# Pasqui1010/DART-Planner

Hardware: AMD Instinct MI355X
Metric: SE(3) rollouts/sec (N=30, batch=8192) + p95 solve ms, at 1/2/4/8 MI355X (higher is better)
Workload: dtype f32

## Files before the change

### dart_planner_amd/capi.py

```python
from __future__ import annotations

import ctypes as C
import math
import os
from typing import Optional

_HERE = os.path.dirname(os.path.abspath(__file__))
DEFAULT_LIBRARY = os.path.join(_HERE, "libse3mpc.so")

SE3MPC_MAX_HORIZON = 64
SE3MPC_MAX_CORRECTIONS = 10
SE3MPC_MAX_SPHERES = 256

STATUS_NAMES = {0: "SE3MPC_OK", -1: "SE3MPC_ERR_NULL", -2: "SE3MPC_ERR_HORIZON", -3: "SE3MPC_ERR_SHAPE",
                -4: "SE3MPC_ERR_PARAM", -5: "SE3MPC_ERR_WORKSPACE", -6: "SE3MPC_ERR_LAUNCH",
                -7: "SE3MPC_ERR_NO_DEVICE"}
TASK_MESSAGES = {1: "CONVERGENCE: NORM OF PROJECTED GRADIENT <= PGTOL",
                 2: "CONVERGENCE: RELATIVE REDUCTION OF F <= FACTR*EPSMCH",
                 3: "STOP: TOTAL NO. OF ITERATIONS REACHED LIMIT",
                 4: "STOP: TOTAL NO. OF F,G EVALUATIONS EXCEEDS LIMIT",
                 5: "ABNORMAL: "}


class Se3mpcLibraryError(RuntimeError):
# ... 285 lines not shown
    "mixer_readback": [_XP, _I, _P, _P, _LL, _P, _P, _P, _P, _P, _P],
    "closed_loop_actuated": [_MP, _CP, _SP, _XP, _I, _I, _D] + _PLAN + [_P, _P, _P, _P, _P, _P, _P, _P, _P, _LL, _P, _LL, _I,
                             C.POINTER(C.c_double * 3), _P, _P, _P, _P, _P, _P, _P],
    "latency_push": [_I, _I, _P, _P, _P, _P, _P, _P, _P, _P, _P, _P, _P, _P, _P, _P],
    "onboard_control": [_OP, _I, _P, _P, _P, _P] + _PLAN + [_P, _P, _P, _P, _P],
    "edge_loop": [_OP, _SP, _I, _I, _D] + _PLAN + [_P, _P, _P, _P, _P, _P, _I, _P, _P, _P, _P, _LL, _I, C.POINTER(C.c_double * 3),
                  _P, _P, _P, _P, _P, _P, _P],
    "monte_carlo": [_PP, _CP, _SP, _I, _I, _I, _D, _P, _P, _LL, _P, _P, _P, _P, _P, _P, _P, _P, _P, _P, _P],
    "monte_carlo_staged": [_PP, _CP, _SP, _MP, _XP, _I, _I, _I, _D, _P, _P, _LL, _P, _P, _P, _P, _P, _P, _P, _P, _P, _LL, _P, _P, _P, _P, _P],
    "mppi_closed_loop": [_PP, _CP, _SP, _I, _I, _I, _D, C.c_uint32, _I, _I, _I, _D, _D, C.c_uint64, C.c_uint32, C.c_uint32, _P, _P, _I, _D, _P, _LL,
                         _P, _P, _P, _P, _P, _P, _P, _P, _P, _P, _P, _P],
    "mppi_closed_loop_staged": [_PP, _CP, _SP, _MP, _XP, _I, _I, _I, _D, C.c_uint32, _I, _I, _I, _D, _D, C.c_uint64, C.c_uint32, C.c_uint32, _P, _P, _I,
                                _D, _P, _LL, _P, _P, _P, _P, _P, _P, _P, _P, _P, _LL, _P, _P, _P, _P, _P, _P, _P],
}
_PLAIN_API = {
    "se3mpc_controller_default_params": (C.c_int, [_CP]),
    "se3mpc_simulator_default_params": (C.c_int, [_SP]),
    "se3mpc_controller_reset": (C.c_int, [_CP, _I, _P, _P]),
    "se3mpc_smoother_default_params": (C.c_int, [_MP]),
    "se3mpc_smoother_reset": (C.c_int, [_I, _P, _P]),
    "se3mpc_mixer_default_params": (C.c_int, [_XP]),
    "se3mpc_mixer_reset": (C.c_int, [_I, _P, _P]),
    "se3mpc_onboard_default_params": (C.c_int, [_OP]),
    "se3mpc_onboard_reset": (C.c_int, [_I, _P, _P]),
    "se3mpc_latency_reset": (C.c_int, [_I, _I, _P, _P]),
    "se3mpc_abi_version": (C.c_int, []),
    "se3mpc_last_error": (C.c_char_p, []),
    "se3mpc_device_count": (C.c_int, []),
    "se3mpc_default_params": (C.c_int, [_PP]),
    "se3mpc_check_params": (C.c_int, [_PP]),
    "se3mpc_set_rollout_variant": (C.c_int, [_I]),
    "se3mpc_set_solver_variant": (C.c_int, [_I]),
    "se3mpc_set_edge_loop_variant": (C.c_int, [_I]),
    "se3mpc_reduce_keys": (C.c_int, [_P, _I, _I, _P, _P]),
    "se3mpc_key_index": (C.c_uint32, [C.c_uint64]),
    "se3mpc_key_cost": (C.c_float, [C.c_uint64]),
    "se3mpc_population_workspace": (C.c_int, [_I, _I]),
    "se3mpc_mppi_split_workspace_bytes": (C.c_size_t, [_I, _I, _I]),
}


def exported_symbols() -> list:
    names = list(_PLAIN_API)
    for base in _TYPED_API:
        names += [f"se3mpc_{base}_f32", f"se3mpc_{base}_f64"]
    for base in _LOOP_TYPED_API:
        names += [f"se3mpc_{base}_f32", f"se3mpc_{base}_f64"]
    names += list(_VOXEL_PLAIN_API)
    for base in _VOXEL_TYPED_API:
        names += [f"se3mpc_voxel_{base}_f32", f"se3mpc_voxel_{base}_f64"]
    return names


class Library:

    def __init__(self, path: Optional[str] = None):
        self.path = path or os.environ.get("SE3MPC_LIBRARY", DEFAULT_LIBRARY)
        if not os.path.exists(self.path):
            raise Se3mpcLibraryError(
                f"{self.path} not found: the HIP extension has not been built.  Run "
                "`python -c 'import __graft_entry__ as g; g.build()'` (or `make -C dart_planner_amd/csrc`). "
                "There is no CPU fallback.")
        try:
            self._dll = C.CDLL(self.path)
        except OSError as e:
            raise Se3mpcLibraryError(f"cannot load {self.path}: {e}") from e
# ... 19 lines not shown
            for suf in ("f32", "f64"):
                fn = getattr(self._dll, f"se3mpc_voxel_{base}_{suf}")
                fn.restype = C.c_int
                fn.argtypes = [_VP] + args
        if self._dll.se3mpc_abi_version() != 1:
            raise Se3mpcLibraryError(f"{self.path}: ABI version {self._dll.se3mpc_abi_version()} != 1")

    def abi_version(self) -> int:
        return self._dll.se3mpc_abi_version()

    def last_error(self) -> str:
        return (self._dll.se3mpc_last_error() or b"").decode()

    def device_count(self) -> int:
        return self._dll.se3mpc_device_count()

    def default_params(self) -> Params:
        p = Params()
        self._check("se3mpc_default_params", self._dll.se3mpc_default_params(C.byref(p)))
        return p

    def check_params(self, p: Params) -> int:
        return self._dll.se3mpc_check_params(C.byref(p))

    def set_rollout_variant(self, variant: int) -> None:
        self._check("se3mpc_set_rollout_variant", self._dll.se3mpc_set_rollout_variant(variant))

    def set_solver_variant(self, variant: int) -> None:
        self._check("se3mpc_set_solver_variant", self._dll.se3mpc_set_solver_variant(variant))

    def set_edge_loop_variant(self, variant: int) -> None:
        self._check("se3mpc_set_edge_loop_variant", self._dll.se3mpc_set_edge_loop_variant(variant))

    def reduce_keys(self, wave_keys: int, per_batch: int, nbatch: int, keys_out: int, stream: int) -> None:
        self._check("se3mpc_reduce_keys", self._dll.se3mpc_reduce_keys(wave_keys, per_batch, nbatch, keys_out, stream))

    def population_workspace(self, rows: int, B: int) -> int:
        return self._dll.se3mpc_population_workspace(rows, B)

    def mppi_split_workspace_bytes(self, horizon: int, nprob: int, splits: int) -> int:
        return self._dll.se3mpc_mppi_split_workspace_bytes(horizon, nprob, splits)

    def key_index(self, key: int) -> int:
        return self._dll.se3mpc_key_index(C.c_uint64(key))

    def key_cost(self, key: int) -> float:
        return self._dll.se3mpc_key_cost(C.c_uint64(key))

    def call(self, base: str, suffix: str, *args, params: Optional[Params] = None) -> None:
        fn = getattr(self._dll, f"se3mpc_{base}_{suffix}")
        has_params = _TYPED_API[base][0]
        if has_params:
            if params is None:
                raise TypeError(f"se3mpc_{base} needs params")
            rc = fn(C.byref(params), *args)
        else:
            rc = fn(*args)
        self._check(f"se3mpc_{base}_{suffix}", rc)

    def call_status(self, base: str, suffix: str, *args, params: Optional[Params] = None) -> int:
        fn = getattr(self._dll, f"se3mpc_{base}_{suffix}")
        if _TYPED_API[base][0]:
            return fn(C.byref(params) if params is not None else None, *args)
        return fn(*args)

    def controller_default_params(self) -> ControllerParams:
# ... 74 lines not shown
```

### dart_planner_amd/csrc/closed_loop.hip

```cpp
#pragma clang fp contract(off)
#include "closed_loop_device.hpp"

namespace se3mpc {

template <typename R>
__global__ void __launch_bounds__(64)
control_kernel(CtrlDev<R> c, int B, const double* __restrict__ time, const R* __restrict__ pos, const R* __restrict__ vel,
               const R* __restrict__ att, const R* __restrict__ omega, const R* __restrict__ dpos, const R* __restrict__ dvel,
               const R* __restrict__ dacc, const R* __restrict__ yaw, const R* __restrict__ yaw_rate, double* __restrict__ state,
               R* __restrict__ thrust, R* __restrict__ torque, R* __restrict__ body_thrust, R* __restrict__ body_rates,
               int32_t* __restrict__ flags, const double* __restrict__ sample_time, PlanView<R> plan, R* __restrict__ target) {
  const int b = blockIdx.x * blockDim.x + threadIdx.x;
  if (b >= B) return;
  CtrlRegs<R> s = load_ctrl<R>(state + (size_t)b * SE3MPC_CONTROLLER_STATE_WORDS);
  DroneRegs<R> d;
  d.load_state(b, pos, vel, att, omega);
  R dp[3], dv[3], da[3];
  if (sample_time != nullptr) {
    const PlanView<R> rows = plan.of(b);
    PlanCursor<R> cur;
    cursor_reset(cur);
    sample_plan<R>(sample_time[b], plan.N, rows.ts, rows.P, rows.V, rows.A, dp, dv, da, cur);
    if (target != nullptr) for (int i = 0; i < 3; ++i) { target[9 * b + i] = dp[i]; target[9 * b + 3 + i] = dv[i]; target[9 * b + 6 + i] = da[i]; }
  } else {
// ... 88 lines not shown
  if (cos_angle != nullptr) cos_angle[b] = ca;
  if (singular != nullptr) singular[b] = sing ? 1 : 0;
}

template <typename R>
__global__ void __launch_bounds__(64)
closed_loop_kernel(CtrlDev<R> c, SimDev<R> m, int B, int nsteps, double sim_dt, PlanView<R> plan, double* __restrict__ time,
                   R* __restrict__ pos, R* __restrict__ vel, R* __restrict__ att, R* __restrict__ omega, double* __restrict__ state,
                   const R* __restrict__ wind, long long wind_stride, int gust_step, R gx, R gy, R gz, int stop_at_plan_end,
                   R* __restrict__ log_state, R* __restrict__ log_cmd, double* __restrict__ log_time, int32_t* __restrict__ steps_taken) {
  const int b = blockIdx.x * blockDim.x + threadIdx.x;
  if (b >= B) return;
  CtrlRegs<R> s = load_ctrl<R>(state + (size_t)b * SE3MPC_CONTROLLER_STATE_WORDS);
  DroneRegs<R> d;
  d.load(b, pos, vel, att, omega, wind, wind_stride, time);
  const int N = plan.N;
  const PlanView<R> rows = plan.of(b);
  const double* __restrict__ ts = rows.ts;
  const R* __restrict__ Pb = rows.P;
  const R* __restrict__ Vb = rows.V;
  const R* __restrict__ Ab = rows.A;
  const R dt = (R)sim_dt;
  PlanCursor<R> cur;
  cursor_reset(cur);
  const int taken = lane_loop<R>(d, b, B, nsteps, gust_step, gx, gy, gz, stop_at_plan_end != 0, ts[N - 1], log_state, log_cmd, log_time,
                                 [&](int, R& th, R* tq) { flight_step<R>(c, m, s, cur, N, ts, Pb, Vb, Ab, d.p, d.v, d.a, d.w, d.t, dt, sim_dt, d.wd, th, tq); });
  d.store(b, pos, vel, att, omega, time);
  store_ctrl<R>(state + (size_t)b * SE3MPC_CONTROLLER_STATE_WORDS, s);
  if (steps_taken != nullptr) steps_taken[b] = taken;
}

template <typename R>
__global__ void __launch_bounds__(64)
simulator_step_kernel(SimDev<R> m, int B, double dt_d, const R* __restrict__ thrust, const R* __restrict__ torque, const R* __restrict__ wind,
                      long long wind_stride, double* __restrict__ time, R* __restrict__ pos, R* __restrict__ vel, R* __restrict__ att,
                      R* __restrict__ omega) {
  const int b = blockIdx.x * blockDim.x + threadIdx.x;
  if (b >= B) return;
  DroneRegs<R> d;
  d.load(b, pos, vel, att, omega, wind, wind_stride, time);
  const R tq[3] = {torque[3 * b], torque[3 * b + 1], torque[3 * b + 2]};
  simulator_step<R>(m, d.p, d.v, d.a, d.w, d.t, thrust[b], tq, (R)dt_d, dt_d, d.wd);
  d.store(b, pos, vel, att, omega, time);
}

__global__ void __launch_bounds__(64)
controller_reset_kernel(int B, double hover, double* __restrict__ state) {
  const int b = blockIdx.x * blockDim.x + threadIdx.x;
  if (b >= B) return;
  double* s = state + (size_t)b * SE3MPC_CONTROLLER_STATE_WORDS;
  for (int i = 0; i < SE3MPC_CONTROLLER_STATE_WORDS; ++i) s[i] = 0.0;
  s[3] = __builtin_nan("");
  s[4] = hover;
}

template <typename R>
int control_impl(const se3mpc_controller_params* cp, int B, const double* time, const R* pos, const R* vel, const R* att, const R* omega,
                 const R* dpos, const R* dvel, const R* dacc, const R* yaw, const R* yaw_rate, double* state, R* thrust, R* torque,
                 R* body_thrust, R* body_rates, int32_t* flags, void* stream) {
  int rc = check_controller_params(cp);
  if (rc) return rc;
  if (B < 0) return SE3MPC_ERR_SHAPE;
  if (B == 0) return SE3MPC_OK;
  if (!time || !pos || !vel || !att || !omega || !dpos || !dvel || !state) return SE3MPC_ERR_NULL;
  hipLaunchKernelGGL(control_kernel<R>, dim3(grid_for(B, 64)), dim3(64), 0, (hipStream_t)stream, make_ctrl_dev<R>(*cp), B, time, pos, vel,
                     att, omega, dpos, dvel, dacc, yaw, yaw_rate, state, thrust, torque, body_thrust, body_rates, flags,
// ... 65 lines not shown
                     b3_des, current_yaw, frame, cos_angle, singular);
  return launch_status("se3mpc_controller_desired_frame");
}

template <typename R>
int control_plan_impl(const se3mpc_controller_params* cp, int B, const double* time, const double* sample_time, const R* pos, const R* vel,
                      const R* att, const R* omega, const PlanView<R>& plan, double* state, R* thrust, R* torque, R* body_thrust,
                      R* body_rates, int32_t* flags, R* target, void* stream) {
  int rc = check_controller_params(cp);
  if (rc) return rc;
  if (B < 0 || !plan_shape_ok(plan, 1)) return SE3MPC_ERR_SHAPE;
  if (B == 0) return SE3MPC_OK;
  if (!time || !sample_time || !pos || !vel || !att || !omega || !plan_present(plan) || !state) return SE3MPC_ERR_NULL;
  hipLaunchKernelGGL(control_kernel<R>, dim3(grid_for(B, 64)), dim3(64), 0, (hipStream_t)stream, make_ctrl_dev<R>(*cp), B, time, pos, vel,
                     att, omega, (const R*)nullptr, (const R*)nullptr, (const R*)nullptr, (const R*)nullptr, (const R*)nullptr, state, thrust,
                     torque, body_thrust, body_rates, flags, sample_time, plan, target);
  return launch_status("se3mpc_control_plan");
}

template <typename R>
int simulator_step_impl(const se3mpc_simulator_params* sp, int B, double dt, const R* thrust, const R* torque, const R* wind,
                        long long wind_stride, double* time, R* pos, R* vel, R* att, R* omega, void* stream) {
  int rc = check_simulator_params(sp);
  if (rc) return rc;
  if (!std::isfinite(dt)) return SE3MPC_ERR_PARAM;
  if (B < 0 || wind_stride < 0) return SE3MPC_ERR_SHAPE;
  if (B == 0) return SE3MPC_OK;
  if (!thrust || !torque || !time || !pos || !vel || !att || !omega) return SE3MPC_ERR_NULL;
  hipLaunchKernelGGL(simulator_step_kernel<R>, dim3(grid_for(B, 64)), dim3(64), 0, (hipStream_t)stream, make_sim_dev<R>(*sp), B, dt, thrust,
                     torque, wind, wind_stride, time, pos, vel, att, omega);
  return launch_status("se3mpc_simulator_step");
}

template <typename R>
int closed_loop_impl(const se3mpc_controller_params* cp, const se3mpc_simulator_params* sp, int B, int nsteps, double sim_dt,
                     const PlanView<R>& plan, double* time, R* pos, R* vel, R* att, R* omega, double* state, const R* wind,
                     long long wind_stride, int gust_step, const double* gust_wind, int stop_at_plan_end, R* log_state, R* log_cmd,
                     double* log_time, int32_t* steps_taken, void* stream) {
  int rc = check_controller_params(cp);
  if (rc) return rc;
  rc = check_simulator_params(sp);
  if (rc) return rc;
  if (!std::isfinite(sim_dt)) return SE3MPC_ERR_PARAM;
  if (B < 0 || nsteps < 0 || !plan_shape_ok(plan, 1) || wind_stride < 0) return SE3MPC_ERR_SHAPE;
  if (B == 0 || nsteps == 0) return SE3MPC_OK;
  if (!plan_present(plan) || !time || !pos || !vel || !att || !omega || !state || (gust_step >= 0 && !gust_wind)) return SE3MPC_ERR_NULL;
  const R gx = gust_step >= 0 ? (R)gust_wind[0] : (R)0, gy = gust_step >= 0 ? (R)gust_wind[1] : (R)0, gz = gust_step >= 0 ? (R)gust_wind[2] : (R)0;
  hipLaunchKernelGGL(closed_loop_kernel<R>, dim3(grid_for(B, 64)), dim3(64), 0, (hipStream_t)stream, make_ctrl_dev<R>(*cp), make_sim_dev<R>(*sp),
                     B, nsteps, sim_dt, plan, time, pos, vel, att, omega, state, wind,
                     wind_stride, gust_step, gx, gy, gz, stop_at_plan_end, log_state, log_cmd, log_time, steps_taken);
  return launch_status("se3mpc_closed_loop");
}

}

using namespace se3mpc;

extern "C" int se3mpc_controller_default_params(se3mpc_controller_params* out) {
  if (out == nullptr) return SE3MPC_ERR_NULL;
  const se3mpc_controller_params d = {{20.0, 20.0, 25.0}, {1.5, 1.5, 2.0}, {10.0, 10.0, 12.0}, {18.0, 18.0, 8.0}, {7.0, 7.0, 3.5},
                                      {0.02, 0.02, 0.04}, {0.5, 0.5, 0.05}, {2.0, 2.0, 3.0},
                                      2.5, M_PI / 4.0, 1.0, 9.80665, 22.0, 0.8, 1.0, 0.6, 0.1, 0.99, 0.95, 0.1, 0.0, 0, 0};
  *out = d;
  return SE3MPC_OK;
}

extern "C" int se3mpc_simulator_default_params(se3mpc_simulator_params* out) {
  if (out == nullptr) return SE3MPC_ERR_NULL;
  const se3mpc_simulator_params d = {1.5, 9.81, {0.1, 0.1, 0.2}, 20.0, 10.0};
  *out = d;
  return SE3MPC_OK;
}

extern "C" int se3mpc_controller_reset(const se3mpc_controller_params* cp, int B, double* state, void* stream) {
  int rc = check_controller_params(cp);
  if (rc) return rc;
  if (B < 0) return SE3MPC_ERR_SHAPE;
  if (B == 0) return SE3MPC_OK;
  if (!state) return SE3MPC_ERR_NULL;
  hipLaunchKernelGGL(controller_reset_kernel, dim3(grid_for(B, 64)), dim3(64), 0, (hipStream_t)stream, B, cp->mass * cp->gravity, state);
  return launch_status("se3mpc_controller_reset");
}

#define SE3MPC_DEFINE_LOOP_API(SUF, R)                                                                                      \
  extern "C" int se3mpc_control_##SUF(const se3mpc_controller_params* cp, int B, const double* time, const R* pos, const R* vel, \
                                      const R* att, const R* omega, const R* dpos, const R* dvel, const R* dacc, const R* yaw, \
                                      const R* yaw_rate, double* state, R* thrust, R* torque, R* body_thrust, R* body_rates,  \
                                      int32_t* flags, void* stream) {                                                       \
    return control_impl<R>(cp, B, time, pos, vel, att, omega, dpos, dvel, dacc, yaw, yaw_rate, state, thrust, torque,       \
                           body_thrust, body_rates, flags, stream);                                                        \
  }                                                                                                                         \
  extern "C" int se3mpc_control_fast_##SUF(const se3mpc_controller_params* cp, double vehicle_mass, double vehicle_gravity, int B,  \
                                           double dt, const R* pos, const R* vel, const R* att, const R* omega, const R* dpos,   \
                                           const R* dvel, const R* dacc, const R* yaw, const R* yaw_rate, double* state, R* thrust, \
                                           R* torque, int32_t* flags, void* stream) {                                          \
    return control_fast_impl<R>(cp, vehicle_mass, vehicle_gravity, B, dt, pos, vel, att, omega, dpos, dvel, dacc, yaw, yaw_rate, \
                                state, thrust, torque, flags, stream);                                                      \
  }                                                                                                                         \
  extern "C" int se3mpc_controller_integral_update_##SUF(const se3mpc_controller_params* cp, int B, const R* vel_error, double dt,   \
                                                         const int32_t* saturation, double* state, void* stream) {             \
    return integral_update_impl<R>(cp, B, vel_error, dt, saturation, state, stream);                                        \
  }                                                                                                                         \
  extern "C" int se3mpc_controller_attitude_torque_##SUF(const se3mpc_controller_params* cp, int B, const R* att, const R* omega,   \
                                                         const R* b3_des, const R* yaw, const R* yaw_rate, const double* inertia, \
                                                         double* state, R* torque, int32_t* flags, void* stream) {           \
    return attitude_torque_impl<R>(cp, B, att, omega, b3_des, yaw, yaw_rate, inertia, state, torque, flags, stream);          \
  }                                                                                                                         \
  extern "C" int se3mpc_controller_desired_frame_##SUF(const se3mpc_controller_params* cp, int B, int method, const R* yaw_vector,  \
                                                       const R* b3_des, const R* current_yaw, R* frame, R* cos_angle,        \
                                                       int32_t* singular, void* stream) {                                   \
    return desired_frame_impl<R>(cp, B, method, yaw_vector, b3_des, current_yaw, frame, cos_angle, singular, stream);         \
  }                                                                                                                         \
  extern "C" int se3mpc_control_plan_##SUF(const se3mpc_controller_params* cp, int B, const double* time, const double* sample_time, \
                                           const R* pos, const R* vel, const R* att, const R* omega, int N, const double* timestamps, \
// ... 27 lines not shown
```

### dart_planner_amd/csrc/closed_loop_device.hpp

```cpp
#pragma once
#include <hip/hip_runtime.h>

#include <cmath>

#include "se3mpc_common.hpp"

static_assert(sizeof(se3mpc_controller_params) == 304, "se3mpc_controller_params is part of the C ABI (capi.py mirrors it)");
static_assert(sizeof(se3mpc_simulator_params) == 56, "se3mpc_simulator_params is part of the C ABI");

namespace se3mpc {

template <typename R>
struct CtrlDev {
  R kp_pos[3], ki_pos[3], kd_pos[3], kp_att[3], kd_att[3], inertia[3], max_torque[3], max_int_axis[3];
  R max_integral_pos, max_tilt, cos_max_tilt, gravity, max_thrust, min_thrust_abs, hover, track_thr, vel_thr, kb, decay, sat_thr,
      yaw_sing_thr, dh_cos, dh_sin;
  int anti_windup, fallback;
};

template <typename R>
static CtrlDev<R> make_ctrl_dev(const se3mpc_controller_params& p) {
  CtrlDev<R> c;
  for (int i = 0; i < 3; ++i) {
    c.kp_pos[i] = (R)p.kp_pos[i]; c.ki_pos[i] = (R)p.ki_pos[i]; c.kd_pos[i] = (R)p.kd_pos[i];
    c.kp_att[i] = (R)p.kp_att[i]; c.kd_att[i] = (R)p.kd_att[i]; c.inertia[i] = (R)p.inertia[i];
    c.max_torque[i] = (R)p.max_torque_xyz[i]; c.max_int_axis[i] = (R)p.max_integral_per_axis[i];
  }
  c.max_integral_pos = (R)p.max_integral_pos; c.max_tilt = (R)p.max_tilt_angle; c.cos_max_tilt = (R)std::cos(p.max_tilt_angle);
  c.gravity = (R)p.gravity; c.max_thrust = (R)p.max_thrust;
  c.min_thrust_abs = (R)(p.min_thrust * p.mass * p.gravity);
  c.hover = (R)(p.mass * p.gravity);
  c.track_thr = (R)p.tracking_error_threshold; c.vel_thr = (R)p.velocity_error_threshold;
  c.kb = (R)p.back_calculation_gain; c.decay = (R)p.integral_decay_factor; c.sat_thr = (R)p.saturation_threshold;
  c.yaw_sing_thr = (R)p.yaw_singularity_threshold;
  c.dh_cos = (R)std::cos(p.default_heading_yaw); c.dh_sin = (R)std::sin(p.default_heading_yaw);
  c.anti_windup = p.anti_windup_method; c.fallback = p.yaw_fallback_method;
  return c;
}
// ... 461 lines not shown
    after_step(step, r.p);
  }
  r.store(d);
  store_ctrl<R>(d.ctrl, s);
}

template <typename R, typename F>
__device__ __forceinline__ int lane_loop(DroneRegs<R>& d, int b, int B, int nsteps, int gust_step, R gx, R gy, R gz, bool stop_at_plan_end,
                                         double ts_last, R* __restrict__ log_state, R* __restrict__ log_cmd, double* __restrict__ log_time,
                                         F&& fly) {
  int taken = 0;
  bool active = true;
  for (int step = 0; step < nsteps; ++step) {
    if (stop_at_plan_end && d.t > ts_last) active = false;
    if (log_state != nullptr) {
      R* ls = log_state + ((size_t)step * B + b) * 12;
      for (int i = 0; i < 3; ++i) { ls[i] = d.p[i]; ls[3 + i] = d.v[i]; ls[6 + i] = d.a[i]; ls[9 + i] = d.w[i]; }
    }
    if (log_time != nullptr) log_time[(size_t)step * B + b] = d.t;
    R th = (R)NAN, tq[3] = {(R)NAN, (R)NAN, (R)NAN};
    if (active) {
      if (step == gust_step) { d.wd[0] = gx; d.wd[1] = gy; d.wd[2] = gz; }
      fly(step, th, tq);
      ++taken;
    }
    if (log_cmd != nullptr) {
      R* lc = log_cmd + ((size_t)step * B + b) * 4;
      lc[0] = th; lc[1] = tq[0]; lc[2] = tq[1]; lc[3] = tq[2];
    }
  }
  return taken;
}

static inline int check_controller_params(const se3mpc_controller_params* p) {
  if (p == nullptr) return SE3MPC_ERR_NULL;
  const double* d = reinterpret_cast<const double*>(p);
  for (int i = 0; i < 37; ++i)
    if (!std::isfinite(d[i])) return SE3MPC_ERR_PARAM;
  if (!(p->mass > 0.0) || p->anti_windup_method < 0 || p->anti_windup_method > 2 || p->yaw_fallback_method < 0 || p->yaw_fallback_method > 3)
    return SE3MPC_ERR_PARAM;
  return SE3MPC_OK;
}

static inline int check_simulator_params(const se3mpc_simulator_params* sp) {
  if (sp == nullptr) return SE3MPC_ERR_NULL;
  if (!(sp->mass > 0.0) || !std::isfinite(sp->gravity) || !(sp->inertia[0] > 0.0) || !(sp->inertia[1] > 0.0) || !(sp->inertia[2] > 0.0) ||
      !std::isfinite(sp->max_thrust) || !std::isfinite(sp->max_torque))
    return SE3MPC_ERR_PARAM;
  return SE3MPC_OK;
}

__device__ __forceinline__ double plan_stamp(int cycle, int substeps, double sim_dt, int k, double dt) {
  const double base = (double)(cycle * substeps) * sim_dt;
  const double off = (double)k * dt;
  return base + off;
}

}
```

### dart_planner_amd/csrc/monte_carlo.hip

```cpp
#include "solve_device.hpp"
#pragma clang fp contract(off)
#include "closed_loop_device.hpp"
#pragma clang fp contract(fast)

namespace se3mpc {

template <typename IO, int G>
__global__ void __launch_bounds__(64, SE3MPC_MC_WAVES)
monte_carlo_kernel(SolveDev q, CtrlDev<IO> ctl, SimDev<IO> sim, int B, int cycles, int substeps, double sim_dt, size_t solver_lds,
                   const IO* __restrict__ goalg, const IO* __restrict__ windg, long long wind_stride, double* __restrict__ timeg,
                   IO* __restrict__ posg, IO* __restrict__ velg, IO* __restrict__ attg, IO* __restrict__ omegag,
                   double* __restrict__ stateg, IO* __restrict__ Xg, IO* __restrict__ accg, se3mpc_solve_info* __restrict__ infog,
                   int* __restrict__ overflowed) {
  HIP_DYNAMIC_SHARED(unsigned char, lds_raw)
  constexpr int P = kWave / G, J = kSlots;
  const int lane = lane_id();
  const int k = lane & (G - 1);
  const int grp = lane / G;
  const int pb = blockIdx.x * P + grp;
  if (pb >= B) return;
  double goal[3] = {0.0, 0.0, 0.0};
  if (q.has_goal) {
#pragma unroll
    for (int a = 0; a < 3; ++a) goal[a] = (double)goalg[pb * 3 + a];
// ... 11 lines not shown
    {
      const IO* s_vec = mc_block<IO, G>(lds_raw, solver_lds, grp).d.vec;
#pragma unroll
      for (int a = 0; a < 3; ++a) { ps[a] = (double)s_vec[a]; vs[a] = (double)s_vec[3 + a]; }
    }
    double x[J];
    {
#include "solve_body.inc"
      if (task == SE3MPC_TASK_OVERFLOW && k == 0) atomicAdd(overflowed, 1);
      const DroneBlock<IO> drone = mc_block<IO, G>(lds_raw, solver_lds, grp).d;
      if (live) {
#pragma unroll
        for (int a = 0; a < 3; ++a) { drone.planP[3 * k + a] = (IO)x[a]; drone.planV[3 * k + a] = (IO)x[3 + a]; }
        drone.planA[3 * k + 0] = (IO)(x[6] / q.mass); drone.planA[3 * k + 1] = (IO)(x[7] / q.mass); drone.planA[3 * k + 2] = (IO)(x[8] / q.mass - q.grav);
        drone.stamps[k] = plan_stamp(cycle, substeps, sim_dt, k, q.dt);
      }
      if (cycle == cycles - 1 && live) {
        if (Xg != nullptr) {
#pragma unroll
          for (int j = 0; j < J; ++j) Xg[(size_t)pb * n + (j / 3) * n3 + 3 * k + (j % 3)] = (IO)x[j];
        }
        if (accg != nullptr) {
          const size_t o = (size_t)pb * n3 + 3 * k;
          accg[o] = drone.planA[3 * k + 0]; accg[o + 1] = drone.planA[3 * k + 1]; accg[o + 2] = drone.planA[3 * k + 2];
        }
        if (infog != nullptr && k == 0) {
          se3mpc_solve_info r;
          r.fun = f; r.nit = nit; r.nfev = nfev; r.status = status; r.task = task;
          infog[pb] = r;
        }
      }
    }
    group_sync<G>();
    if (k == 0) {
      const McBlock<IO> blk = mc_block<IO, G>(lds_raw, solver_lds, grp);
      const CtrlDev<IO> c = *blk.ctl;
      const SimDev<IO> m = *blk.sim;
      fly_steps<IO>(c, m, blk.d, q.N, substeps, sim_dt, [](int, const IO*) {});
    }
    group_sync<G>();
  }
  if (k == 0) drone_store<IO>(mc_block<IO, G>(lds_raw, solver_lds, grp).d, pb, posg, velg, attg, omegag, timeg, stateg);
}

template <typename IO>
int monte_carlo_impl(const se3mpc_params* p, const se3mpc_controller_params* cp, const se3mpc_simulator_params* sp, int B, int cycles,
                     int substeps, double sim_dt, const IO* goal, const IO* wind, long long wind_stride, double* time, IO* pos, IO* vel,
                     IO* att, IO* omega, double* state, IO* X_last, IO* acc_last, se3mpc_solve_info* info_last, int32_t* overflowed,
                     void* stream) {
  if (p == nullptr || cp == nullptr || sp == nullptr) return SE3MPC_ERR_NULL;
  int rc = check_params_impl(p);
  if (rc) return rc;
  rc = check_controller_params(cp);
  if (rc) return rc;
  rc = check_simulator_params(sp);
  if (rc) return rc;
  if (B < 0 || cycles < 0 || substeps < 0 || p->horizon > kWave) return SE3MPC_ERR_SHAPE;
  if (!std::isfinite(sim_dt)) return SE3MPC_ERR_PARAM;
  if (wind != nullptr && !(wind_stride == 0 || wind_stride >= 3)) return SE3MPC_ERR_SHAPE;
  if (B == 0) return SE3MPC_OK;
  if (!time || !pos || !vel || !att || !omega || !state || !overflowed || (p->has_goal && !goal)) return SE3MPC_ERR_NULL;
  hipStream_t s = (hipStream_t)stream;
  if (hipMemsetAsync(overflowed, 0, sizeof(int32_t), s) != hipSuccess) return launch_status("se3mpc_monte_carlo(memset)");
  SolveDev q = make_solve_dev(*p);
  const int G = solve_group_for_horizon(p->horizon);
  const int waves = (int)(((long)B * G + kWave - 1) / kWave);
  const size_t extra = (size_t)(kWave / G) * mc_group_bytes<IO>(G);
  const size_t per_cu = (size_t)(waves + 255) / 256;
  const size_t budget = (size_t)160 * 1024 / (per_cu < 1 ? 1 : (per_cu > 8 ? 8 : per_cu));
  int mlds = q.m;
  while (mlds > 4 && solve_lds_bytes(mlds, G, sizeof(IO)) + extra > budget) --mlds;
// ... 34 lines not shown
```

### include/se3mpc.h

```cpp
#ifndef SE3MPC_H
#define SE3MPC_H

#include <stddef.h>
#include <stdint.h>

#ifdef __cplusplus
extern "C" {
#endif

#define SE3MPC_ABI_VERSION 1
#define SE3MPC_MAX_HORIZON 64
#define SE3MPC_MAX_CORRECTIONS 10
#define SE3MPC_MAX_SPHERES 256

enum se3mpc_status {
  SE3MPC_OK = 0,
  SE3MPC_ERR_NULL = -1,
  SE3MPC_ERR_HORIZON = -2,
  SE3MPC_ERR_SHAPE = -3,
  SE3MPC_ERR_PARAM = -4,
  SE3MPC_ERR_WORKSPACE = -5,
  SE3MPC_ERR_LAUNCH = -6,
  SE3MPC_ERR_NO_DEVICE = -7
};
// ... 496 lines not shown
int se3mpc_latency_push_f32(int B, int depth, const double* time, const float* pos, const float* vel, const float* att,
                            const float* omega, float* ring, double* ring_time, double* state, double* d_time, float* d_pos, float* d_vel,
                            float* d_att, float* d_omega, void* stream);
int se3mpc_latency_push_f64(int B, int depth, const double* time, const double* pos, const double* vel, const double* att,
                            const double* omega, double* ring, double* ring_time, double* state, double* d_time, double* d_pos,
                            double* d_vel, double* d_att, double* d_omega, void* stream);

int se3mpc_onboard_control_f32(const se3mpc_onboard_params* op, int B, const double* time, const float* pos, const float* att,
                               const float* omega, int N, const double* timestamps, long long ts_stride, const float* P, long long strideP,
                               const float* V, long long strideV, const float* A, long long strideA, double* state, float* thrust,
                               float* torque, float* target_pos, void* stream);
int se3mpc_onboard_control_f64(const se3mpc_onboard_params* op, int B, const double* time, const double* pos, const double* att,
                               const double* omega, int N, const double* timestamps, long long ts_stride, const double* P,
                               long long strideP, const double* V, long long strideV, const double* A, long long strideA, double* state,
                               double* thrust, double* torque, double* target_pos, void* stream);

int se3mpc_edge_loop_f32(const se3mpc_onboard_params* op, const se3mpc_simulator_params* sp, int B, int nsteps, double sim_dt, int N,
                         const double* timestamps, long long ts_stride, const float* P, long long strideP, const float* V,
                         long long strideV, const float* A, long long strideA, double* time, float* pos, float* vel, float* att,
                         float* omega, double* onboard_state, int depth, float* ring, double* ring_time, double* latency_state,
                         const float* wind, long long wind_stride, int gust_step, const double* gust_wind, float* log_state,
                         float* log_cmd, double* log_time, float* log_target, double* log_delayed_time, int32_t* zero_thrust_steps,
                         void* stream);
int se3mpc_edge_loop_f64(const se3mpc_onboard_params* op, const se3mpc_simulator_params* sp, int B, int nsteps, double sim_dt, int N,
                         const double* timestamps, long long ts_stride, const double* P, long long strideP, const double* V,
                         long long strideV, const double* A, long long strideA, double* time, double* pos, double* vel, double* att,
                         double* omega, double* onboard_state, int depth, double* ring, double* ring_time, double* latency_state,
                         const double* wind, long long wind_stride, int gust_step, const double* gust_wind, double* log_state,
                         double* log_cmd, double* log_time, double* log_target, double* log_delayed_time, int32_t* zero_thrust_steps,
                         void* stream);

int se3mpc_set_edge_loop_variant(int variant);

int se3mpc_set_solver_variant(int variant);

int se3mpc_solve_f32(const se3mpc_params* p, int B, const float* p0, const float* v0, const float* goal,
                     const float* x0, float* X, se3mpc_solve_info* info, float* acc, float* att,
                     float* rates, float* thrust, void* stream);
int se3mpc_solve_f64(const se3mpc_params* p, int B, const double* p0, const double* v0, const double* goal,
                     const double* x0, double* X, se3mpc_solve_info* info, double* acc, double* att,
                     double* rates, double* thrust, void* stream);

int se3mpc_plan_host_f32(const se3mpc_params* p, int B, const float* p0, const float* v0, const float* goal,
                         const float* x0, float* X, se3mpc_solve_info* info, float* acc, float* att, float* rates,
                         float* thrust, unsigned long long* done, unsigned long long ticket, double timeout_us, void* stream);
int se3mpc_plan_host_f64(const se3mpc_params* p, int B, const double* p0, const double* v0, const double* goal,
                         const double* x0, double* X, se3mpc_solve_info* info, double* acc, double* att, double* rates,
                         double* thrust, unsigned long long* done, unsigned long long ticket, double timeout_us, void* stream);

#ifdef __cplusplus
}
#endif
#endif
```

Before: 8.035 billion.

## Split per-drone closed-loop controller across a quad of lanes using DPP

Adds a quad-lane variant of the closed-loop controller and simulator. Each drone is handled by four lanes, one per axis plus a spare, and cross-axis norms, cross products and broadcasts use DPP quad permutes. It is the default for batches up to a threshold and is also used in the Monte Carlo block's fly steps, where four lanes now fly instead of one. The intent is more parallelism for the serial per-drone control loop. In exchange it adds DPP traffic, wastes a lane on rotations, and redundantly reloads parameters per lane.

```diff
diff --git a/dart_planner_amd/capi.py b/dart_planner_amd/capi.py
--- a/dart_planner_amd/capi.py
+++ b/dart_planner_amd/capi.py
@@ -341,6 +341,7 @@
     "se3mpc_set_rollout_variant": (C.c_int, [_I]),
     "se3mpc_set_solver_variant": (C.c_int, [_I]),
     "se3mpc_set_edge_loop_variant": (C.c_int, [_I]),
+    "se3mpc_set_closed_loop_variant": (C.c_int, [_I]),
     "se3mpc_reduce_keys": (C.c_int, [_P, _I, _I, _P, _P]),
     "se3mpc_key_index": (C.c_uint32, [C.c_uint64]),
     "se3mpc_key_cost": (C.c_float, [C.c_uint64]),
@@ -426,6 +427,9 @@
     def set_edge_loop_variant(self, variant: int) -> None:
         self._check("se3mpc_set_edge_loop_variant", self._dll.se3mpc_set_edge_loop_variant(variant))
 
+    def set_closed_loop_variant(self, variant: int) -> None:
+        self._check("se3mpc_set_closed_loop_variant", self._dll.se3mpc_set_closed_loop_variant(variant))
+
     def reduce_keys(self, wave_keys: int, per_batch: int, nbatch: int, keys_out: int, stream: int) -> None:
         self._check("se3mpc_reduce_keys", self._dll.se3mpc_reduce_keys(wave_keys, per_batch, nbatch, keys_out, stream))
 
diff --git a/dart_planner_amd/csrc/closed_loop.hip b/dart_planner_amd/csrc/closed_loop.hip
--- a/dart_planner_amd/csrc/closed_loop.hip
+++ b/dart_planner_amd/csrc/closed_loop.hip
@@ -144,6 +144,35 @@
 
 template <typename R>
 __global__ void __launch_bounds__(64)
+closed_loop_quad_kernel(CtrlDev<R> c, SimDev<R> m, int B, int nsteps, double sim_dt, PlanView<R> plan, double* __restrict__ time,
+                        R* __restrict__ pos, R* __restrict__ vel, R* __restrict__ att, R* __restrict__ omega, double* __restrict__ state,
+                        const R* __restrict__ wind, long long wind_stride, int gust_step, R gx, R gy, R gz, int stop_at_plan_end,
+                        R* __restrict__ log_state, R* __restrict__ log_cmd, double* __restrict__ log_time, int32_t* __restrict__ steps_taken) {
+  const int b = (int)(blockIdx.x * (blockDim.x >> 2) + (threadIdx.x >> 2));
+  if (b >= B) return;
+  const QuadAxis<R> x = make_quad_axis<R>(c, m);
+  QuadCtrlRegs<R> s = load_ctrl<R>(state + (size_t)b * SE3MPC_CONTROLLER_STATE_WORDS, x);
+  QuadDroneRegs<R> d;
+  d.load(b, x.ax, pos, vel, att, omega, wind, wind_stride, time);
+  const int N = plan.N;
+  const PlanView<R> rows = plan.of(b);
+  const double* __restrict__ ts = rows.ts;
+  const R* __restrict__ Pb = rows.P;
+  const R* __restrict__ Vb = rows.V;
+  const R* __restrict__ Ab = rows.A;
+  const R dt = (R)sim_dt;
+  QuadPlanCursor<R> cur;
+  cursor_reset(cur);
+  const int taken = lane_loop_quad<R>(d, x, b, B, nsteps, gust_step, gx, gy, gz, stop_at_plan_end != 0, ts[N - 1], log_state, log_cmd, log_time,
+                                      [&](int, R& th, R& tq) { flight_step<R>(c, m, x, s, cur, N, ts, Pb, Vb, Ab, d, dt, sim_dt, th, tq); });
+  quad_sync();
+  d.store(b, x.lane, pos, vel, att, omega, time);
+  store_ctrl<R>(state + (size_t)b * SE3MPC_CONTROLLER_STATE_WORDS, s, x);
+  if (steps_taken != nullptr && x.lane == 0) steps_taken[b] = taken;
+}
+
+template <typename R>
+__global__ void __launch_bounds__(64)
 simulator_step_kernel(SimDev<R> m, int B, double dt_d, const R* __restrict__ thrust, const R* __restrict__ torque, const R* __restrict__ wind,
                       long long wind_stride, double* __restrict__ time, R* __restrict__ pos, R* __restrict__ vel, R* __restrict__ att,
                       R* __restrict__ omega) {
@@ -275,6 +304,12 @@
   return launch_status("se3mpc_simulator_step");
 }
 
+static int g_closed_loop_variant = 0;
+constexpr int kClosedLoopQuadMaxDrones = 16384;
+static inline bool closed_loop_on_quads(int B) {
+  return g_closed_loop_variant == 2 || (g_closed_loop_variant == 0 && B <= kClosedLoopQuadMaxDrones);
+}
+
 template <typename R>
 int closed_loop_impl(const se3mpc_controller_params* cp, const se3mpc_simulator_params* sp, int B, int nsteps, double sim_dt,
                      const PlanView<R>& plan, double* time, R* pos, R* vel, R* att, R* omega, double* state, const R* wind,
@@ -289,9 +324,14 @@
   if (B == 0 || nsteps == 0) return SE3MPC_OK;
   if (!plan_present(plan) || !time || !pos || !vel || !att || !omega || !state || (gust_step >= 0 && !gust_wind)) return SE3MPC_ERR_NULL;
   const R gx = gust_step >= 0 ? (R)gust_wind[0] : (R)0, gy = gust_step >= 0 ? (R)gust_wind[1] : (R)0, gz = gust_step >= 0 ? (R)gust_wind[2] : (R)0;
-  hipLaunchKernelGGL(closed_loop_kernel<R>, dim3(grid_for(B, 64)), dim3(64), 0, (hipStream_t)stream, make_ctrl_dev<R>(*cp), make_sim_dev<R>(*sp),
-                     B, nsteps, sim_dt, plan, time, pos, vel, att, omega, state, wind,
-                     wind_stride, gust_step, gx, gy, gz, stop_at_plan_end, log_state, log_cmd, log_time, steps_taken);
+  if (closed_loop_on_quads(B))
+    hipLaunchKernelGGL(closed_loop_quad_kernel<R>, dim3(grid_for(B, 16)), dim3(64), 0, (hipStream_t)stream, make_ctrl_dev<R>(*cp),
+                       make_sim_dev<R>(*sp), B, nsteps, sim_dt, plan, time, pos, vel, att, omega, state, wind,
+                       wind_stride, gust_step, gx, gy, gz, stop_at_plan_end, log_state, log_cmd, log_time, steps_taken);
+  else
+    hipLaunchKernelGGL(closed_loop_kernel<R>, dim3(grid_for(B, 64)), dim3(64), 0, (hipStream_t)stream, make_ctrl_dev<R>(*cp), make_sim_dev<R>(*sp),
+                       B, nsteps, sim_dt, plan, time, pos, vel, att, omega, state, wind,
+                       wind_stride, gust_step, gx, gy, gz, stop_at_plan_end, log_state, log_cmd, log_time, steps_taken);
   return launch_status("se3mpc_closed_loop");
 }
 
@@ -323,6 +363,12 @@
   if (!state) return SE3MPC_ERR_NULL;
   hipLaunchKernelGGL(controller_reset_kernel, dim3(grid_for(B, 64)), dim3(64), 0, (hipStream_t)stream, B, cp->mass * cp->gravity, state);
   return launch_status("se3mpc_controller_reset");
+}
+
+extern "C" int se3mpc_set_closed_loop_variant(int variant) {
+  if (variant < 0 || variant > 2) return reject(SE3MPC_ERR_PARAM, "se3mpc_set_closed_loop_variant: 0, 1 or 2");
+  g_closed_loop_variant = variant;
+  return SE3MPC_OK;
 }
 
 #define SE3MPC_DEFINE_LOOP_API(SUF, R)                                                                                      \
diff --git a/dart_planner_amd/csrc/closed_loop_device.hpp b/dart_planner_amd/csrc/closed_loop_device.hpp
--- a/dart_planner_amd/csrc/closed_loop_device.hpp
+++ b/dart_planner_amd/csrc/closed_loop_device.hpp
@@ -4,6 +4,7 @@
 #include <cmath>
 
 #include "se3mpc_common.hpp"
+#include <se3mpc_quad_ops.hpp>
 
 static_assert(sizeof(se3mpc_controller_params) == 304, "se3mpc_controller_params is part of the C ABI (capi.py mirrors it)");
 static_assert(sizeof(se3mpc_simulator_params) == 56, "se3mpc_simulator_params is part of the C ABI");
@@ -531,6 +532,350 @@
   return taken;
 }
 
+template <typename T>
+__device__ __forceinline__ T pick3(int ax, T x, T y, T z) { return ax == 0 ? x : (ax == 1 ? y : z); }
+template <typename R>
+__device__ __forceinline__ R quad_sum(R v) { return (quad_bcast<0>(v) + quad_bcast<1>(v)) + quad_bcast<2>(v); }
+template <typename R>
+__device__ __forceinline__ R quad_norm(R v) { return sqrt(quad_sum(v * v)); }
+template <typename R>
+__device__ __forceinline__ R quad_cross(R a, R b) { return quad_rot1(a) * quad_rot2(b) - quad_rot2(a) * quad_rot1(b); }
+
+template <typename R>
+struct QuadAxis {
+  int lane, ax;
+  R kp_pos, ki_pos, kd_pos, kp_att, kd_att, inertia, max_torque, max_int_axis, sim_inertia;
+  R unit_x;
+  R bc_share;
+  R sim_gravity;
+};
+template <typename R>
+__device__ __forceinline__ QuadAxis<R> make_quad_axis(const CtrlDev<R>& c, const SimDev<R>& m) {
+  QuadAxis<R> x;
+  x.lane = quad_lane();
+  x.ax = x.lane < 2 ? x.lane : 2;
+  x.kp_pos = pick3(x.ax, c.kp_pos[0], c.kp_pos[1], c.kp_pos[2]); x.ki_pos = pick3(x.ax, c.ki_pos[0], c.ki_pos[1], c.ki_pos[2]);
+  x.kd_pos = pick3(x.ax, c.kd_pos[0], c.kd_pos[1], c.kd_pos[2]); x.kp_att = pick3(x.ax, c.kp_att[0], c.kp_att[1], c.kp_att[2]);
+  x.kd_att = pick3(x.ax, c.kd_att[0], c.kd_att[1], c.kd_att[2]); x.inertia = pick3(x.ax, c.inertia[0], c.inertia[1], c.inertia[2]);
+  x.max_torque = pick3(x.ax, c.max_torque[0], c.max_torque[1], c.max_torque[2]);
+  x.max_int_axis = pick3(x.ax, c.max_int_axis[0], c.max_int_axis[1], c.max_int_axis[2]);
+  x.sim_inertia = pick3(x.ax, m.inertia[0], m.inertia[1], m.inertia[2]);
+  x.unit_x = x.ax == 0 ? (R)1 : (R)0;
+  x.bc_share = x.ax == 2 ? (R)0.34 : (R)0.33;
+  x.sim_gravity = x.ax == 2 ? -m.gravity : (R)0;
+  return x;
+}
+
+template <typename R>
+struct QuadCtrlRegs {
+  R integral;
+  double last_time;
+  R last_valid_thrust, unsat_thrust, unsat_torque;
+  int failsafe_count, halvings;
+  int flags;
+  bool torque_sat;
+};
+template <typename R>
+__device__ __forceinline__ QuadCtrlRegs<R> load_ctrl(const double* __restrict__ s, const QuadAxis<R>& x) {
+  QuadCtrlRegs<R> r;
+  r.integral = (R)s[x.ax]; r.unsat_torque = (R)s[6 + x.ax];
+  r.last_time = s[3]; r.last_valid_thrust = (R)s[4]; r.unsat_thrust = (R)s[5];
+  r.failsafe_count = (int)s[9]; r.halvings = (int)s[10];
+  const int fl = (int)s[11];
+  r.flags = fl & ~(4 | 8 | 16);
+  r.torque_sat = (fl & (4 << x.ax)) != 0;
+  return r;
+}
+template <typename R>
+__device__ __forceinline__ void store_ctrl(double* __restrict__ s, const QuadCtrlRegs<R>& r, const QuadAxis<R>& x) {
+  const int ts = r.torque_sat ? 1 : 0;
+  const int fl = r.flags | (quad_bcast<0>(ts) << 2) | (quad_bcast<1>(ts) << 3) | (quad_bcast<2>(ts) << 4);
+  if (x.lane < 3) { s[x.ax] = (double)r.integral; s[6 + x.ax] = (double)r.unsat_torque; }
+  if (x.lane == 0) {
+    s[3] = r.last_time; s[4] = (double)r.last_valid_thrust; s[5] = (double)r.unsat_thrust;
+    s[9] = (double)r.failsafe_count; s[10] = (double)r.halvings; s[11] = (double)fl;
+  }
+}
+
+template <typename R>
+__device__ __forceinline__ void enter_failsafe(QuadCtrlRegs<R>& s) {
+  if (!(s.flags & 1)) {
+    s.halvings += 1;
+    s.integral = (R)0;
+    s.failsafe_count += 1;
+  }
+  s.flags |= 1;
+}
+
+template <typename R>
+__device__ __forceinline__ void update_integral(const CtrlDev<R>& c, const QuadAxis<R>& x, QuadCtrlRegs<R>& s, R ve, R dt, bool thrust_sat) {
+  R upd = ve * dt;
+  if (c.anti_windup == 0) {
+    if (thrust_sat) upd = upd * (R)0.1;
+    if (s.torque_sat) upd = upd * (R)0.1;
+  } else if (c.anti_windup == 1) {
+    if (thrust_sat) {
+      const R fb = (s.unsat_thrust - c.max_thrust) * c.kb;
+      upd = upd - fb * x.bc_share;
+    }
+    if (s.torque_sat) upd = upd - ((s.unsat_torque - x.max_torque) * c.kb) * (R)0.5;
+  }
+  R I = s.integral + upd;
+  if (fabs(I) > x.max_int_axis) I = sign_of(I) * x.max_int_axis;
+  const R mag = quad_norm(I);
+  if (mag > c.max_integral_pos) { const R f = c.max_integral_pos / mag; I = I * f; }
+  if (fabs(I) > x.max_int_axis * c.sat_thr) I = I * c.decay;
+  s.integral = I;
+}
+
+template <typename R>
+__device__ __forceinline__ void desired_frame(const CtrlDev<R>& c, const QuadAxis<R>& x, R yv, R b3n, R cy, R sy, R& b1, R& b2) {
+  const R cos_angle = fabs(quad_sum(yv * b3n));
+  const int method = c.fallback;
+  if (cos_angle >= c.yaw_sing_thr) {
+    R proj = x.unit_x - quad_bcast<0>(b3n) * b3n;
+    const R np_ = quad_norm(proj);
+    proj = proj / np_;
+    if (method == 1 || method == 2) {
+      const R hv = pick3(x.ax, method == 1 ? c.dh_cos : cy, method == 1 ? c.dh_sin : sy, (R)0);
+      const R cx = quad_cross(hv, b3n);
+      const R nc = quad_norm(cx);
+      if (nc > (R)1e-6) b1 = cx / nc;
+      else b1 = proj;
+    } else if (method != 0 || fabs(quad_bcast<2>(b3n)) < (R)0.99) {
+      b1 = proj;
+    } else {
+      b1 = x.unit_x;
+    }
+  } else {
+    b1 = quad_cross(yv, b3n);
+    const R n1 = quad_norm(b1);
+    if (n1 > (R)1e-6) b1 = b1 / n1;
+    else b1 = x.unit_x;
+  }
+  b2 = quad_cross(b3n, b1);
+}
+
+template <typename R>
+__device__ __forceinline__ R attitude_torque(const CtrlDev<R>& c, const QuadAxis<R>& x, QuadCtrlRegs<R>& s, R scale, R b3, R att, R omega,
+                                             R yaw_des, R yaw_rate_des) {
+  R sn, cs;
+  sin_cos(x.lane == 3 ? yaw_des : att, sn, cs);
+  const R sr = quad_bcast<0>(sn), cr = quad_bcast<0>(cs), sp = quad_bcast<1>(sn), cp = quad_bcast<1>(cs);
+  const R sy = quad_bcast<2>(sn), cy = quad_bcast<2>(cs), ys = quad_bcast<3>(sn), yc = quad_bcast<3>(cs);
+  const R u = x.ax == 0 ? cy : sy, w = x.ax == 0 ? sy : cy;
+  const R usp = u * sp, wcr = w * cr, wsr = w * sr;
+  const R m1a = usp * sr, m2a = usp * cr;
+  const R Rm0 = x.ax == 2 ? -sp : u * cp;
+  const R Rm1 = x.ax == 2 ? cp * sr : (x.ax == 0 ? m1a - wcr : m1a + wcr);
+  const R Rm2 = x.ax == 2 ? cp * cr : (x.ax == 0 ? m2a + wsr : m2a - wsr);
+  const R yv = pick3(x.ax, yc, ys, (R)0);
+  const R n3 = quad_norm(b3);
+  const R b3n = b3 / n3;
+  R b1, b2;
+  desired_frame(c, x, yv, b3n, cy, sy, b1, b2);
+  const R d0 = quad_sum(b3n * Rm1) - quad_sum(Rm2 * b2);
+  const R d1 = quad_sum(b1 * Rm2) - quad_sum(Rm0 * b3n);
+  const R d2 = quad_sum(b2 * Rm0) - quad_sum(Rm1 * b1);
+  const R eR = (R)0.5 * pick3(x.ax, d0, d1, d2);
+  const R eO = x.ax == 2 ? omega - yaw_rate_des : omega;
+  const R Iw = x.inertia * omega;
+  const R cor = quad_cross(omega, Iw);
+  R tq = (-(x.kp_att * scale) * eR - (x.kd_att * scale) * eO) + cor;
+  s.unsat_torque = tq;
+  s.torque_sat = fabs(tq) > x.max_torque;
+  if (s.torque_sat) tq = sign_of(tq) * x.max_torque;
+  return tq;
+}
+
+template <typename R>
+__device__ __forceinline__ R attitude_command(const CtrlDev<R>& c, const QuadAxis<R>& x, QuadCtrlRegs<R>& s, R scale, R tvw, R tm, R att, R omega,
+                                              R yaw_des, R yaw_rate_des) {
+  R b3;
+  if (tm > (R)1e-6) b3 = tvw / tm;
+  else b3 = x.ax == 2 ? (R)1 : (R)0;
+  const R b3z = quad_bcast<2>(b3);
+  if (fmin(fmax(b3z, (R)-1), (R)1) < c.cos_max_tilt) {
+    const R sf = c.cos_max_tilt / b3z;
+    b3 = x.ax == 2 ? c.cos_max_tilt : b3 * sf;
+    const R n = quad_norm(b3);
+    b3 = b3 / n;
+  }
+  return attitude_torque(c, x, s, scale, b3, att, omega, yaw_des, yaw_rate_des);
+}
+
+template <typename R>
+__device__ __forceinline__ void control_step(const CtrlDev<R>& c, const QuadAxis<R>& x, QuadCtrlRegs<R>& s, double t, R pos, R vel, R att, R omega,
+                                             R dpos, R dvel, R dacc, R yaw_des, R yaw_rate_des, R& thrust_out, R& torque_out) {
+  const double dt_d = (s.last_time != s.last_time) ? 0.001 : t - s.last_time;
+  s.last_time = t;
+  if (dt_d <= 0.0 || dt_d > 0.1) {
+    enter_failsafe(s);
+    thrust_out = s.last_valid_thrust; torque_out = (R)0;
+    return;
+  }
+  const R dt = (R)dt_d;
+  const R scale = (R)ldexp(1.0, -s.halvings);
+  const R pe = dpos - pos, ve = dvel - vel;
+  const R pen = quad_norm(pe), ven = quad_norm(ve);
+  const R acc_pid = ((x.kp_pos * scale) * pe + (x.kd_pos * scale) * ve) + x.ki_pos * s.integral;
+  R tvw = dacc + acc_pid;
+  tvw = x.ax == 2 ? tvw + c.gravity : tvw;
+  R tm = quad_norm(tvw);
+  s.unsat_thrust = tm;
+  bool thrust_sat = false;
+  if (tm > c.max_thrust) { tm = c.max_thrust; thrust_sat = true; }
+  else if (tm < c.min_thrust_abs) { tm = c.min_thrust_abs; thrust_sat = true; }
+  s.flags = (s.flags & ~2) | (thrust_sat ? 2 : 0);
+  update_integral(c, x, s, ve, dt, thrust_sat);
+  if (pen > c.track_thr && ven > c.vel_thr) s.failsafe_count += 1;
+  else s.failsafe_count = s.failsafe_count > 1 ? s.failsafe_count - 1 : 0;
+  if (s.failsafe_count > 100) {
+    enter_failsafe(s);
+    thrust_out = s.last_valid_thrust; torque_out = (R)0;
+    return;
+  }
+  torque_out = attitude_command(c, x, s, scale, tvw, tm, att, omega, yaw_des, yaw_rate_des);
+  s.last_valid_thrust = tm;
+  s.flags &= ~1;
+  s.failsafe_count = 0;
+  thrust_out = tm;
+}
+
+template <typename R>
+struct QuadPlanCursor {
+  int idx, rows_of;
+  double t1, t2;
+  R r1[3], r2[3];
+};
+template <typename R>
+__device__ __forceinline__ void cursor_reset(QuadPlanCursor<R>& c) { c.idx = 0; c.rows_of = -1; }
+template <typename R>
+__device__ __forceinline__ void cursor_before_step(QuadPlanCursor<R>& cur, double sim_dt) {
+  if (!(sim_dt > 0.0)) cur.idx = 0;
+}
+
+template <typename R>
+__device__ __forceinline__ void sample_plan(double t, int N, const double* __restrict__ ts, const R* __restrict__ P, const R* __restrict__ V,
+                                            const R* __restrict__ A, int ax, R tg[3], QuadPlanCursor<R>& c) {
+  int idx = c.idx;
+  while (idx < N && ts[idx] < t) ++idx;
+  c.idx = idx;
+  if (idx != c.rows_of) {
+    const int i1 = idx == 0 ? 0 : (idx >= N ? N - 1 : idx - 1), i2 = idx >= N ? N - 1 : idx;
+    c.t1 = ts[i1]; c.t2 = ts[i2];
+    c.r1[0] = P[3 * i1 + ax]; c.r2[0] = P[3 * i2 + ax];
+    c.r1[1] = V != nullptr ? V[3 * i1 + ax] : (R)0; c.r2[1] = V != nullptr ? V[3 * i2 + ax] : (R)0;
+    c.r1[2] = A != nullptr ? A[3 * i1 + ax] : (R)0; c.r2[2] = A != nullptr ? A[3 * i2 + ax] : (R)0;
+    c.rows_of = idx;
+  }
+  if (idx == 0 || idx >= N) {
+    for (int j = 0; j < 3; ++j) tg[j] = c.r1[j];
+    return;
+  }
+  const R f = (R)((t - c.t1) / (c.t2 - c.t1));
+  for (int j = 0; j < 3; ++j) tg[j] = c.r1[j] + f * (c.r2[j] - c.r1[j]);
+}
+
+template <typename R>
+struct QuadDroneRegs {
+  R p, v, a, w, wd;
+  double t;
+  __device__ __forceinline__ void load(int b, int ax, const R* __restrict__ pos, const R* __restrict__ vel, const R* __restrict__ att,
+                                       const R* __restrict__ omega, const R* __restrict__ wind, long long wind_stride,
+                                       const double* __restrict__ time) {
+    p = pos[3 * b + ax]; v = vel[3 * b + ax]; a = att[3 * b + ax]; w = omega[3 * b + ax];
+    wd = wind != nullptr ? wind[(size_t)b * wind_stride + ax] : (R)0;
+    t = time[b];
+  }
+  __device__ __forceinline__ void store(int b, int lane, R* __restrict__ pos, R* __restrict__ vel, R* __restrict__ att, R* __restrict__ omega,
+                                        double* __restrict__ time) const {
+    if (lane < 3) { pos[3 * b + lane] = p; vel[3 * b + lane] = v; att[3 * b + lane] = a; omega[3 * b + lane] = w; }
+    if (lane == 0) time[b] = t;
+  }
+  __device__ __forceinline__ void load(const DroneBlock<R>& d, int ax) {
+    p = d.vec[ax]; v = d.vec[3 + ax]; a = d.vec[6 + ax]; w = d.vec[9 + ax]; wd = d.vec[12 + ax];
+    t = *d.time;
+  }
+  __device__ __forceinline__ void store(const DroneBlock<R>& d, int lane) const {
+    if (lane < 3) { d.vec[lane] = p; d.vec[3 + lane] = v; d.vec[6 + lane] = a; d.vec[9 + lane] = w; }
+    if (lane == 0) *d.time = t;
+  }
+};
+
+template <typename R>
+__device__ __forceinline__ void simulator_step(const SimDev<R>& m, const QuadAxis<R>& x, QuadDroneRegs<R>& d, R thrust, R torque, R dt, double dt_d) {
+  thrust = fmin(fmax(thrust, (R)0), m.max_thrust);
+  const R tq = fmin(fmax(torque, -m.max_torque), m.max_torque);
+  const R wind_accel = d.wd / m.mass;
+  const R lift = thrust / m.mass;
+  const R acc = (x.sim_gravity + (x.ax == 2 ? lift : (R)0)) + wind_accel;
+  d.v = d.v + acc * dt;
+  d.p = d.p + d.v * dt;
+  const R ang_acc = tq / x.sim_inertia;
+  d.w = d.w + ang_acc * dt;
+  d.a = d.a + d.w * dt;
+  d.t = d.t + dt_d;
+}
+
+template <typename R>
+__device__ __forceinline__ void flight_step(const CtrlDev<R>& c, const SimDev<R>& m, const QuadAxis<R>& x, QuadCtrlRegs<R>& s, QuadPlanCursor<R>& cur,
+                                            int N, const double* ts, const R* P, const R* V, const R* A, QuadDroneRegs<R>& d, R dt, double sim_dt,
+                                            R& th, R& tq) {
+  R tg[3];
+  cursor_before_step(cur, sim_dt);
+  sample_plan<R>(d.t, N, ts, P, V, A, x.ax, tg, cur);
+  control_step<R>(c, x, s, d.t, d.p, d.v, d.a, d.w, tg[0], tg[1], tg[2], (R)0, (R)0, th, tq);
+  simulator_step<R>(m, x, d, th, tq, dt, sim_dt);
+}
+
+template <typename R>
+__device__ __forceinline__ void fly_steps_quad(const CtrlDev<R> c, const SimDev<R> m, const DroneBlock<R>& d, int N, int n, double sim_dt) {
+  const QuadAxis<R> x = make_quad_axis<R>(c, m);
+  QuadCtrlRegs<R> s = load_ctrl<R>(d.ctrl, x);
+  QuadDroneRegs<R> r;
+  r.load(d, x.ax);
+  const R dt = (R)sim_dt;
+  QuadPlanCursor<R> cur;
+  cursor_reset(cur);
+  for (int step = 0; step < n; ++step) {
+    R th, tq;
+    flight_step<R>(c, m, x, s, cur, N, d.stamps, d.planP, d.planV, d.planA, r, dt, sim_dt, th, tq);
+  }
+  quad_sync();
+  r.store(d, x.lane);
+  store_ctrl<R>(d.ctrl, s, x);
+}
+
+template <typename R, typename F>
+__device__ __forceinline__ int lane_loop_quad(QuadDroneRegs<R>& d, const QuadAxis<R>& x, int b, int B, int nsteps, int gust_step, R gx, R gy, R gz,
+                                              bool stop_at_plan_end, double ts_last, R* __restrict__ log_state, R* __restrict__ log_cmd,
+                                              double* __restrict__ log_time, F&& fly) {
+  int taken = 0;
+  bool active = true;
+  const R gust = pick3(x.ax, gx, gy, gz);
+  for (int step = 0; step < nsteps; ++step) {
+    if (stop_at_plan_end && d.t > ts_last) active = false;
+    if (log_state != nullptr && x.lane < 3) {
+      R* ls = log_state + ((size_t)step * B + b) * 12;
+      ls[x.lane] = d.p; ls[3 + x.lane] = d.v; ls[6 + x.lane] = d.a; ls[9 + x.lane] = d.w;
+    }
+    if (log_time != nullptr && x.lane == 0) log_time[(size_t)step * B + b] = d.t;
+    R th = (R)NAN, tq = (R)NAN;
+    if (active) {
+      if (step == gust_step) d.wd = gust;
+      fly(step, th, tq);
+      ++taken;
+    }
+    if (log_cmd != nullptr) {
+      R* lc = log_cmd + ((size_t)step * B + b) * 4;
+      if (x.lane == 0) lc[0] = th;
+      if (x.lane < 3) lc[1 + x.lane] = tq;
+    }
+  }
+  return taken;
+}
+
 static inline int check_controller_params(const se3mpc_controller_params* p) {
   if (p == nullptr) return SE3MPC_ERR_NULL;
   const double* d = reinterpret_cast<const double*>(p);
diff --git a/dart_planner_amd/csrc/monte_carlo.hip b/dart_planner_amd/csrc/monte_carlo.hip
--- a/dart_planner_amd/csrc/monte_carlo.hip
+++ b/dart_planner_amd/csrc/monte_carlo.hip
@@ -67,11 +67,11 @@
       }
     }
     group_sync<G>();
-    if (k == 0) {
+    if (k < 4) {
       const McBlock<IO> blk = mc_block<IO, G>(lds_raw, solver_lds, grp);
       const CtrlDev<IO> c = *blk.ctl;
       const SimDev<IO> m = *blk.sim;
-      fly_steps<IO>(c, m, blk.d, q.N, substeps, sim_dt, [](int, const IO*) {});
+      fly_steps_quad<IO>(c, m, blk.d, q.N, substeps, sim_dt);
     }
     group_sync<G>();
   }
diff --git a/dart_planner_amd/csrc/se3mpc_quad_ops.hpp b/dart_planner_amd/csrc/se3mpc_quad_ops.hpp
--- /dev/null
+++ b/dart_planner_amd/csrc/se3mpc_quad_ops.hpp
@@ -0,0 +1,40 @@
+#pragma once
+#include <hip/hip_runtime.h>
+#include <stdint.h>
+
+namespace se3mpc {
+
+constexpr int kDppQuadBcast0 = 0x00;
+constexpr int kDppQuadBcast1 = 0x55;
+constexpr int kDppQuadBcast2 = 0xAA;
+constexpr int kDppQuadBcast3 = 0xFF;
+constexpr int kDppQuadRot1 = 0xC9;
+constexpr int kDppQuadRot2 = 0xD2;
+
+template <int CTRL>
+__device__ __forceinline__ int quad_dpp(int v) { return __builtin_amdgcn_mov_dpp(v, CTRL, 0xF, 0xF, true); }
+template <int CTRL>
+__device__ __forceinline__ float quad_dpp(float v) { return __int_as_float(quad_dpp<CTRL>(__float_as_int(v))); }
+template <int CTRL>
+__device__ __forceinline__ double quad_dpp(double v) {
+  const uint64_t x = (uint64_t)__double_as_longlong(v);
+  const uint32_t lo = (uint32_t)quad_dpp<CTRL>((int)(uint32_t)x);
+  const uint32_t hi = (uint32_t)quad_dpp<CTRL>((int)(uint32_t)(x >> 32));
+  return __longlong_as_double((long long)(((uint64_t)hi << 32) | lo));
+}
+
+template <int J, typename T>
+__device__ __forceinline__ T quad_bcast(T v) {
+  static_assert(J >= 0 && J < 4, "lane of a quad");
+  return quad_dpp<J * 0x55>(v);
+}
+template <typename T>
+__device__ __forceinline__ T quad_rot1(T v) { return quad_dpp<kDppQuadRot1>(v); }
+template <typename T>
+__device__ __forceinline__ T quad_rot2(T v) { return quad_dpp<kDppQuadRot2>(v); }
+
+__device__ __forceinline__ void quad_sync() { __builtin_amdgcn_wave_barrier(); }
+
+__device__ __forceinline__ int quad_lane() { return (int)(threadIdx.x & 3u); }
+
+}
diff --git a/include/se3mpc.h b/include/se3mpc.h
--- a/include/se3mpc.h
+++ b/include/se3mpc.h
@@ -552,6 +552,8 @@
 
 int se3mpc_set_edge_loop_variant(int variant);
 
+int se3mpc_set_closed_loop_variant(int variant);
+
 int se3mpc_set_solver_variant(int variant);
 
 int se3mpc_solve_f32(const se3mpc_params* p, int B, const float* p0, const float* v0, const float* goal,
```

Result: no change. 8.001 billion (-0.4%).
